# cserteGT3/RANSAC.jl

Measured on AMD Instinct MI355X. Metric: candidates_scored_per_sec, higher is better.
Workload: dtype f64; 1 GPU; cfg3: 10M-point 40-primitive cloud, 30% outliers, r=32 subsets, B=4096 candidates/GPU/step; points=10000000, subset_points=312500, score_mode=f64, parallelism=candidate-sharded x1, int32 sum all-reduce

## Files before the change

include/ransac_hip_diag.h:

```cpp
#ifndef RANSAC_HIP_DIAG_H
#define RANSAC_HIP_DIAG_H

#include "ransac_hip.h"

#ifdef __cplusplus
extern "C" {
#endif

int rh_dbg_cls_audit(rh_cloud *c, const rh_shape *shapes, int32_t b, const rh_params *p, double *out );
int rh_dbg_cls_soundness(rh_cloud *c, const rh_shape *shapes, int32_t b, const rh_params *p, uint64_t *out );
int rh_dbg_cls_soundness_tiles(rh_cloud *c, const rh_shape *shapes, int32_t b, const rh_params *p, uint64_t *out );
int rh_dbg_cls_soundness_nsig(rh_cloud *c, const rh_shape *shapes, int32_t b, const rh_params *p, uint64_t *out );
int rh_dbg_nsig(const rh_shape *shape, const rh_params *p, double M, double Nm, double Ln, int f32, uint32_t *mask_out ,
                const double *dirs, int64_t ndirs, int32_t *cells_out);
int rh_dbg_group_boxes(rh_cloud *c, double *out, int64_t cap, int64_t *ngroups_out);
int rh_dbg_cylbox(const rh_shape *shape, const rh_params *p, double M, double Nm, int f32, const double *boxes, int64_t n,
                  uint8_t *skip_out, uint8_t *ball_out, float *fields_out );
int rh_dbg_cls_round(const rh_shape *shape, const rh_params *p, double M, double Nm, int f32, int64_t n, const double *xyz,
                     const double *nrm, float *ua_out, float *ub_out, float *rec_out , double *dbg4_out );
int rh_dbg_conebox(const rh_shape *shape, const rh_params *p, double M, double Nm, int f32, const double *boxes, int64_t n,
                   uint8_t *skip_out, float *fields_out );
int rh_dbg_cls_cone(const rh_shape *shape, const rh_params *p, double M, double Nm, int f32, int64_t n, const double *xyz,
                    const double *nrm, int device, float *ua_out, float *ub_out, uint8_t *near_out, float *rec_out ,
                    double *dbg4_out );
int rh_dbg_oct_search_selftest(int64_t n, uint64_t seed, int64_t queries, int64_t *mismatches);

int rh_dbg_enabled_events(const uint8_t *events, int64_t nseq, int32_t len, uint16_t *answers);

int rh_dbg_s4_stats(rh_cloud *c, int mode, uint64_t *out );

typedef struct { int64_t slot; int32_t level; int32_t pad; rh_shape shape; } rh_dbg_cand;
int rh_dbg_sample_fit(rh_cloud *c, const rh_params *p, uint64_t seed, int64_t k0, int32_t n_iters, const double *P_or_null,
                      int32_t rank, int32_t world, rh_dbg_cand *out, int32_t cap, int32_t *n_out, uint64_t *draws_out,
                      int32_t *gave_up_out, int32_t *info_out );

int rh_dbg_wave_keys(const uint32_t *keys, const uint8_t *act, const int32_t *slot, int32_t n, int32_t nslots, int u32, int device,
                     int32_t *sum_out , int32_t *minlead_out , int32_t *scal_out );

#ifdef __cplusplus
}
#endif
#endif
```

ransac.jl_amd/_lib.py:

```python
import ctypes as C
import os

_HERE = os.path.dirname(os.path.abspath(__file__))
SO_PATH = os.path.join(_HERE, "libransac_hip.so")
SO_PATH_DIAG = os.path.join(_HERE, "libransac_hip_diag.so")
OPTION_UNSET = -(1 << 63)
SCORE_PATH = {"auto": 0, "brute": 1, "groups": 2}
REFIT_PATH = {"auto": 0, "scan": 1, "culled": 2}

PLANE, SPHERE, CYLINDER, CONE = 0, 1, 2, 3
KIND_NAMES = {PLANE: "plane", SPHERE: "sphere", CYLINDER: "cylinder", CONE: "cone"}
SCORE_INT64_WRAP, SCORE_F64 = 0, 1
S_LENGTHC, S_ALLCAND, S_NOFMINSET = 1, 2, 3
RH_OK, RH_E_INVALID, RH_E_NODEVICE, RH_E_NOMEM, RH_E_CAPACITY, RH_E_INTERNAL = 0, -1, -2, -3, -4, -5


class Shape(C.Structure):
    _fields_ = [("kind", C.c_int32), ("outwards", C.c_int32), ("v", C.c_double * 10)]


class Params(C.Structure):
    _fields_ = [
        ("eps", C.c_double * 4), ("alpha", C.c_double * 4), ("cos_alpha", C.c_double * 4),
        ("collin_threshold", C.c_double), ("parallelthrdeg", C.c_double), ("cos_parallelthr", C.c_double),
# ... 165 lines not shown
    "rh_mp_allgather": (C.c_int, [_vp, _vp, C.c_int64, _vp]),
    "rh_ransac_mp": (C.c_int, [_vp, C.POINTER(C.c_double), C.POINTER(C.c_double), C.POINTER(Params), C.POINTER(Rng), _vp, C.POINTER(Result)]),
    "rh_dev_free": (C.c_int, [_vp, _vp]),
    "rh_dev_upload": (C.c_int, [_vp, _vp, _vp, C.c_int64]),
    "rh_dev_download": (C.c_int, [_vp, _vp, _vp, C.c_int64]),
    "rh_octree_build": (C.c_int, [_dp, C.c_int64, C.POINTER(C.c_void_p)]),
    "rh_octree_build_f32": (C.c_int, [C.POINTER(C.c_float), C.c_int64, C.POINTER(C.c_void_p)]),
    "rh_octree_destroy": (C.c_int, [_vp]),
    "rh_octree_info": (C.c_int, [_vp, _i32p, _i32p, _i32p]),
    "rh_octree_findleaf": (C.c_int, [_vp, _dp, _i32p]),
    "rh_octree_getnthcell": (C.c_int, [_vp, C.c_int32, C.c_int32, _i32p]),
    "rh_octree_node_info": (C.c_int, [_vp, C.c_int32, _dp, _dp, _i32p, _i32p, _i32p, C.POINTER(C.c_int64)]),
    "rh_octree_node_points": (C.c_int, [_vp, C.c_int32, C.POINTER(C.c_int64), C.c_int64]),
    "rh_octree_cell_enabled": (C.c_int, [_vp, _vp, C.c_int32, C.POINTER(C.c_int64), C.c_int64, C.POINTER(C.c_int64)]),
    "rh_set_option": (C.c_int, [_vp, C.c_char_p, C.c_int64]),
    "rh_get_option": (C.c_int, [_vp, C.c_char_p, _i64p, _i32p]),
    "rh_score_launch_info": (C.c_int, [_vp, C.POINTER(C.c_int32)]),
    "rh_last_list_launch_ms": (C.c_int, [_vp, C.POINTER(C.c_float)]),
    "rh_build_variant": (C.c_int, []),
    "rh_cloud_create_ms": (C.c_int, [_vp, _dp]),
    "rh_comm_unique_id": (C.c_int, [_vp]),
    "rh_comm_create": (C.c_int, [_vp, C.c_int32, C.c_int32, _vp, C.POINTER(_vp)]),
    "rh_comm_destroy": (C.c_int, [_vp]),
    "rh_score_batch_allreduce_dev": (C.c_int, [_vp, _vp, _vp, C.c_int32, C.c_int32, C.c_int32, _pp, _vp]),
    "rh_comm_fence": (C.c_int, [_vp, _vp]),
    "rh_comm_sync": (C.c_int, [_vp]),
    "rh_shape_extents": (C.c_int, [_vp, _sp, C.c_int32, _i64p, _i64p, C.POINTER(Extent)]),
    "rh_shape_extents_dev": (C.c_int, [_vp, _vp, C.c_int32, _vp, _vp, C.c_int64, _vp]),
    "rh_result_extents": (C.c_int, [_vp, C.POINTER(Result), C.POINTER(Extent)]),
    "rh_assign_points": (C.c_int, [_dp, _dp, C.c_int64, _sp, C.c_int32, _pp, C.c_int32, C.c_int, _i32p, _dp, _i64p, _i64p, _i64p]),
    "rh_assign_points_f32": (C.c_int, [C.POINTER(C.c_float), C.POINTER(C.c_float), C.c_int64, _sp, C.c_int32, _pp, C.c_int32, C.c_int,
                                       _i32p, _dp, _i64p, _i64p, _i64p]),
    "rh_cloud_assign": (C.c_int, [_vp, _sp, C.c_int32, _pp, C.c_int32, _i32p, _dp, _i64p, _i64p, _i64p]),
    "rh_cloud_assign_dev": (C.c_int, [_vp, _vp, C.c_int32, _pp, C.c_int32, _vp, _vp, _vp, _vp, _vp]),
    "rh_estimate_normals": (C.c_int, [_dp, C.c_int64, C.POINTER(NormalsParams), _dp, C.c_int, _dp, _dp, _i32p]),
    "rh_estimate_normals_f32": (C.c_int, [C.POINTER(C.c_float), C.c_int64, C.POINTER(NormalsParams), C.POINTER(C.c_float),
                                          C.c_int, C.POINTER(C.c_float), C.POINTER(C.c_float), _i32p]),
    "rh_cluster": (C.c_int, [_dp, C.c_int64, C.POINTER(ClusterParams), C.c_int, _i32p, _u8p, C.c_int64, _i64p, _i64p, _i64p, _i64p,
                             C.POINTER(ClusterStats)]),
    "rh_cluster_f32": (C.c_int, [C.POINTER(C.c_float), C.c_int64, C.POINTER(ClusterParams), C.c_int, _i32p, _u8p, C.c_int64, _i64p,
                                 _i64p, _i64p, _i64p, C.POINTER(ClusterStats)]),
    "rh_orient_normals": (C.c_int, [_dp, _dp, C.c_int64, C.POINTER(OrientParams), C.c_int, _dp, _i32p, _i32p, C.POINTER(OrientStats)]),
    "rh_orient_normals_f32": (C.c_int, [C.POINTER(C.c_float), C.POINTER(C.c_float), C.c_int64, C.POINTER(OrientParams), C.c_int,
                                        C.POINTER(C.c_float), _i32p, _i32p, C.POINTER(OrientStats)]),
    "rh_voxel_downsample": (C.c_int, [_dp, _dp, C.c_int64, C.POINTER(VoxelParams), C.c_int, _dp, _dp, _i64p, _i32p, C.c_int64,
                                      _i32p, _i64p, _i64p]),
    "rh_voxel_downsample_f32": (C.c_int, [C.POINTER(C.c_float), C.POINTER(C.c_float), C.c_int64, C.POINTER(VoxelParams), C.c_int,
                                          C.POINTER(C.c_float), C.POINTER(C.c_float), _i64p, _i32p, C.c_int64, _i32p, _i64p, _i64p]),
    "rh_knn": (C.c_int, [_dp, C.c_int64, C.c_int32, C.c_double, C.c_int, _i32p, _dp, _i32p]),
    "rh_knn_f32": (C.c_int, [C.POINTER(C.c_float), C.c_int64, C.c_int32, C.c_double, C.c_int, _i32p, _dp, _i32p]),
    "rh_knn_query": (C.c_int, [_dp, C.c_int64, _dp, C.c_int64, C.c_int32, C.c_double, C.c_int, _i32p, _dp, _i32p]),
    "rh_knn_query_f32": (C.c_int, [C.POINTER(C.c_float), C.c_int64, C.POINTER(C.c_float), C.c_int64, C.c_int32, C.c_double, C.c_int,
                                   _i32p, _dp, _i32p]),
    "rh_cloud_distance": (C.c_int, [_dp, _dp, C.c_int64, _dp, C.c_int64, C.POINTER(DistanceParams), C.c_int, _dp, _i32p,
                                    C.POINTER(DistanceStats)]),
    "rh_cloud_distance_f32": (C.c_int, [C.POINTER(C.c_float), C.POINTER(C.c_float), C.c_int64, C.POINTER(C.c_float), C.c_int64,
                                        C.POINTER(DistanceParams), C.c_int, _dp, _i32p, C.POINTER(DistanceStats)]),
    "rh_register": (C.c_int, [_dp, _dp, C.c_int64, _dp, C.c_int64, C.POINTER(RegisterParams), _dp, C.c_int, _dp,
                              C.POINTER(RegisterResult), _i32p, _dp]),
    "rh_register_f32": (C.c_int, [C.POINTER(C.c_float), C.POINTER(C.c_float), C.c_int64, C.POINTER(C.c_float), C.c_int64,
                                  C.POINTER(RegisterParams), _dp, C.c_int, _dp, C.POINTER(RegisterResult), _i32p, _dp]),
    "rh_remove_outliers": (C.c_int, [_dp, C.c_int64, C.POINTER(OutlierParams), C.c_int, _u8p, _i32p, C.c_int64, _i64p, _dp,
                                     C.POINTER(OutlierStats)]),
    "rh_remove_outliers_f32": (C.c_int, [C.POINTER(C.c_float), C.c_int64, C.POINTER(OutlierParams), C.c_int, _u8p, _i32p,
                                         C.c_int64, _i64p, _dp, C.POINTER(OutlierStats)]),
}

class DbgCand(C.Structure):
    _fields_ = [("slot", C.c_int64), ("level", C.c_int32), ("pad", C.c_int32), ("shape", Shape)]


DIAG_SIGNATURES = {
    "rh_dbg_sample_fit": (C.c_int, [_vp, _pp, C.c_uint64, C.c_int64, C.c_int32, _dp, C.c_int32, C.c_int32, C.POINTER(DbgCand),
                                    C.c_int32, _i32p, _u64p, _i32p, _i32p]),
    "rh_dbg_cls_audit": (C.c_int, [_vp, _sp, C.c_int32, _pp, _dp]),
    "rh_dbg_cls_soundness": (C.c_int, [_vp, _sp, C.c_int32, _pp, C.POINTER(C.c_uint64)]),
    "rh_dbg_cls_soundness_tiles": (C.c_int, [_vp, _sp, C.c_int32, _pp, C.POINTER(C.c_uint64)]),
    "rh_dbg_cls_soundness_nsig": (C.c_int, [_vp, _sp, C.c_int32, _pp, C.POINTER(C.c_uint64)]),
    "rh_dbg_nsig": (C.c_int, [_sp, _pp, C.c_double, C.c_double, C.c_double, C.c_int, C.POINTER(C.c_uint32), _dp, C.c_int64, _i32p]),
    "rh_dbg_group_boxes": (C.c_int, [_vp, _dp, C.c_int64, C.POINTER(C.c_int64)]),
    "rh_dbg_cylbox": (C.c_int, [_sp, _pp, C.c_double, C.c_double, C.c_int, _dp, C.c_int64, C.POINTER(C.c_uint8), C.POINTER(C.c_uint8), C.POINTER(C.c_float)]),
    "rh_dbg_cls_round": (C.c_int, [_sp, _pp, C.c_double, C.c_double, C.c_int, C.c_int64, _dp, _dp, C.POINTER(C.c_float), C.POINTER(C.c_float),
                                   C.POINTER(C.c_float), _dp]),
    "rh_dbg_conebox": (C.c_int, [_sp, _pp, C.c_double, C.c_double, C.c_int, _dp, C.c_int64, C.POINTER(C.c_uint8), C.POINTER(C.c_float)]),
    "rh_dbg_cls_cone": (C.c_int, [_sp, _pp, C.c_double, C.c_double, C.c_int, C.c_int64, _dp, _dp, C.c_int, C.POINTER(C.c_float),
                                  C.POINTER(C.c_float), C.POINTER(C.c_uint8), C.POINTER(C.c_float), _dp]),
    "rh_dbg_oct_search_selftest": (C.c_int, [C.c_int64, C.c_uint64, C.c_int64, C.POINTER(C.c_int64)]),
    "rh_dbg_enabled_events": (C.c_int, [_u8p, C.c_int64, C.c_int32, C.POINTER(C.c_uint16)]),
    "rh_dbg_s4_stats": (C.c_int, [_vp, C.c_int, C.POINTER(C.c_uint64)]),
    "rh_dbg_wave_keys": (C.c_int, [C.POINTER(C.c_uint32), _u8p, _i32p, C.c_int32, C.c_int32, C.c_int, C.c_int, _i32p, _i32p, _i32p]),
}

_libs = {}


def variant():
    v = os.environ.get("RH_LIB_VARIANT", "product")
    if v not in ("product", "diag"):
        raise RuntimeError("RH_LIB_VARIANT=%r: expected 'product' or 'diag'" % v)
    return v


def _share_torch_hip_runtime():
    import sys
    if "torch" in sys.modules or os.environ.get("RH_SYSTEM_HIP"):
        return
    try:
        import importlib.util
        spec = importlib.util.find_spec("torch")
        if spec is None or not spec.submodule_search_locations:
            return
        path = os.path.join(list(spec.submodule_search_locations)[0], "lib", "libamdhip64.so")
        if os.path.exists(path):
            C.CDLL(path, mode=C.RTLD_GLOBAL)
    except (ImportError, OSError, ValueError):
        pass


def lib(which=None):
    which = which or variant()
    L = _libs.get(which)
    if L is None:
        path = SO_PATH if which == "product" else SO_PATH_DIAG
        if os.environ.get("RH_LIB_PATH"):
            path = os.environ["RH_LIB_PATH"]
        if not os.path.exists(path):
            raise RuntimeError(
                "%s is missing: the HIP extension has not been built and this package has no CPU "
                "fallback (build it with ransac.jl_amd/build.py)" % path)
        _share_torch_hip_runtime()
        L = C.CDLL(path)
        sigs = dict(SIGNATURES)
        if which == "diag":
            sigs.update(DIAG_SIGNATURES)
        for name, (res, args) in sigs.items():
            f = getattr(L, name)
            f.restype = res
            f.argtypes = args
        if L.rh_build_variant() != (1 if which == "diag" else 0):
            raise RuntimeError("%s is not the %s build" % (path, which))
        _libs[which] = L
    return L


def check(rc):
    if rc != RH_OK:
        raise RansacHipError(rc, lib().rh_last_error().decode("utf-8", "replace"))
    return rc
```

ransac.jl_amd/csrc/score4.hip:

```cpp
#include <stdio.h>
#include <stdlib.h>

#include <vector>

#include "rh_internal.h"
#ifdef RH_DIAG
#include "ransac_hip_diag.h"
#endif
#include "score_device.h"
#include "score4_device.h"
#include "wave_keys.h"

namespace {

using namespace rhdev;
using namespace rh4;

typedef float rh_f32x4 __attribute__((ext_vector_type(4)));
typedef float rh_f32x2 __attribute__((ext_vector_type(2)));
typedef unsigned long long rh_u64x2 __attribute__((ext_vector_type(2)));
typedef uint32_t rh_u32x4 __attribute__((ext_vector_type(4)));

constexpr int S4_TG = 4;
constexpr int S4_GB = 2;
// ... 48 lines not shown
    int64_t stcap;
};

#ifdef RH_DIAG
#define S4_STAT(stats, idx, val) do { const unsigned long long v_ = (unsigned long long)(val); if ((stats) != nullptr && (threadIdx.x & 63) == 0) atomicAdd((stats) + (idx), v_); } while (0)
#else
#define S4_STAT(stats, idx, val) do { } while (0)
#endif

template <int KIND> struct S4Fields { static constexpr int NBOX = KIND == RH_PLANE ? 8 : (KIND == RH_SPHERE ? 5 : (KIND == RH_CYLINDER ? 10 : 11)); };

static __device__ __forceinline__ bool nsig_meet(const float (&B)[RH_BOX_FIELDS], const rh_u32x4 gm)
{
    return (((__builtin_bit_cast(uint32_t, B[5]) & gm.x) | (__builtin_bit_cast(uint32_t, B[6]) & gm.y)) | (__builtin_bit_cast(uint32_t, B[7]) & gm.z)) != 0u;
}

#define RH4_CONST_AS __attribute__((address_space(4)))

static __device__ __forceinline__ int wave_shr1(int v) { return __builtin_amdgcn_update_dpp(0, v, 0x138, 0xf, 0xf, false); }
static __device__ __forceinline__ int wave_shl1(int v) { return __builtin_amdgcn_update_dpp(0, v, 0x130, 0xf, 0xf, false); }

static __device__ __forceinline__ int run_total(int v, int key, int lane)
{
    static_assert(S4_TG <= 4, "two steps cover runs of four");
    const int k1 = wave_shr1(key), u1 = wave_shr1(v);
    v += (lane >= 1 && k1 == key) ? u1 : 0;
    const int k2 = wave_shr1(k1), u2 = wave_shr1(wave_shr1(v));
    v += (lane >= 2 && k2 == key) ? u2 : 0;
    const int kn = wave_shl1(key);
    return (lane == 63 || kn != key) ? v : 0;
}

template <int KIND, int R, bool MASK, bool F32, bool LIST>
static __device__ __forceinline__ void
score4_batch(S4Shared<R, MASK, LIST> &sh, const int wv, const int lane, const int head, const int n, const int cbase, const double *__restrict__ pts,
             int64_t stride, const int64_t p0, const rh_prep *__restrict__ prep, const rh_cls *__restrict__ cls,
             const int32_t *__restrict__ orig, double eps, double cosa, int32_t *__restrict__ counts, const bool weird,
             uint64_t *__restrict__ masks, uint8_t *__restrict__ occ, const int64_t mstride, const int64_t g0, unsigned long long *__restrict__ stats)
{
    (void)stats;
    S4_STAT(stats, 24 * KIND + 8, 1);
    const bool act = lane < n;
    const uint32_t e = sh.plist[head + (act ? lane : 0)];
    const int g = (int)(e & S4_GM), ci = LIST ? (int)sh.ctab[e >> S4_GB] : cbase + (int)(e >> S4_GB);
    const rh_f32x4 *__restrict__ rowa = &sh.pa[g][0];
    const rh_f32x2 *__restrict__ rowb = &sh.pb[g][0];
    const rh_cls *__restrict__ rec = &cls[ci];
    int total = 0;
    uint64_t word = 0;
    int qbh = 0, qbn = 0;
    auto drain_b = [&](int k) {
        wave_lds_sync();
        const bool on = lane < k;
        const unsigned e2 = on ? sh.qb[wv][(qbh + lane) & 127] : 0u;
        const int slot = (int)(e2 >> 6);
        const uint32_t pe = sh.plist[head + slot];
        const int64_t gi = p0 + (int)(pe & S4_GM) * 64 + (int)(e2 & 63u);
        uint64_t r;
        if (F32) {
            const rh_prepf Pv = prepf_of<KIND>(prep[LIST ? (int)sh.ctab[pe >> S4_GB] : cbase + (int)(pe >> S4_GB)]);
            const rh_f32x4 a = sh.pa[pe & S4_GM][e2 & 63u];
            const rh_f32x2 b = sh.pb[pe & S4_GM][e2 & 63u];
            r = test_point<KIND>(Pv, a.x, a.y, a.z, a.w, b.x, b.y, eps, cosa);
        } else {
            const rh_prep Pv = prep[LIST ? (int)sh.ctab[pe >> S4_GB] : cbase + (int)(pe >> S4_GB)];
            r = test_point<KIND>(Pv, pts[gi], pts[stride + gi], pts[2 * stride + gi], pts[3 * stride + gi], pts[4 * stride + gi],
                                 pts[5 * stride + gi], eps, cosa);
        }
        S4_STAT(stats, 24 * KIND + (k == 64 ? 11 : 12), 1);
        S4_STAT(stats, 24 * KIND + 13, __popcll(r & (k >= 64 ? ~0ULL : ((1ULL << k) - 1ULL))));
        if (on && ((r >> lane) & 1ULL)) {
            atomicAdd(&sh.cntb[wv][slot], 1);
            if (MASK) atomicOr(&sh.maskb[wv][slot], 1ULL << (e2 & 63u));
        }
        qbh = (qbh + k) & 127;
        qbn -= k;
    };
    if (KIND != RH_CONE) {
        constexpr int NF = KIND == RH_PLANE ? 9 : (KIND == RH_SPHERE ? 8 : 11);
        rh_cls C;
#pragma unroll
        for (int f = 0; f < NF; f++) C.f[f] = rec->f[f];
        const bool exact_only = weird || is_nan_bits(rec->f[RH_CLS_FLAG]);
        uint32_t wlo = 0, whi = 0, umin = 0xffffffffu;
        auto point_u = [&](int j) {
            const rh_f32x4 a = rowa[j];
            const rh_f32x2 b = rowb[j];
            const float u = KIND == RH_PLANE ? cls_plane_u(C, a.x, a.y, a.z, a.w, b.x, b.y)
                                             : cls_round_u<KIND == RH_PLANE ? RH_SPHERE : KIND>(C, a.x, a.y, a.z, a.w, b.x, b.y);
            const uint32_t ub = __builtin_bit_cast(uint32_t, u);
            umin = umin < ub ? umin : ub;
            return ub;
        };
#pragma unroll 8
        for (int j = 0; j < 32; j++) wlo = __builtin_amdgcn_alignbit(wlo, point_u(j), 31);
#pragma unroll 8
        for (int j = 32; j < 64; j++) whi = __builtin_amdgcn_alignbit(whi, point_u(j), 31);
        if (MASK) { wlo = __brev(wlo); whi = __brev(whi); }
        const int cs = __popc(wlo) + __popc(whi);
        const bool amb = act && (umin <= 0x3f800000u || exact_only);
        total = (act && !amb) ? cs : 0;
        word = (act && !amb) ? (((uint64_t)whi << 32) | wlo) : 0ULL;
        uint64_t redo = WB(amb);
        S4_STAT(stats, 24 * KIND + 9, __popcll(redo));
        if (redo != 0) {
            sh.cntb[wv][lane] = 0;
            if (MASK) sh.maskb[wv][lane] = 0ULL;
            while (redo != 0) {
                const int k = __builtin_ctzll(redo);
                redo &= redo - 1;
                const uint32_t ek = __builtin_amdgcn_readlane(e, k);
                const int g2 = (int)(ek & S4_GM);
                const int ci2 = LIST ? __builtin_amdgcn_readfirstlane((int)sh.ctab[ek >> S4_GB]) : cbase + (int)(ek >> S4_GB);
                const RH4_CONST_AS rh_cls *rk = (const RH4_CONST_AS rh_cls *)(uintptr_t)&cls[ci2];
                rh_cls Ck;
#pragma unroll
                for (int f = 0; f < NF; f++) Ck.f[f] = rk->f[f];
                const bool xo = weird || is_nan_bits(rk->f[RH_CLS_FLAG]);
                const rh_f32x4 a = sh.pa[g2][lane];
                const rh_f32x2 b = sh.pb[g2][lane];
                const float u = KIND == RH_PLANE ? cls_plane_u(Ck, a.x, a.y, a.z, a.w, b.x, b.y)
                                                 : cls_round_u<KIND == RH_PLANE ? RH_SPHERE : KIND>(Ck, a.x, a.y, a.z, a.w, b.x, b.y);
                const uint64_t lg = sh.len[g2];
                const uint64_t sure = xo ? 0ULL : (WB(cls_sure(u)) & lg);
                const uint64_t und = xo ? lg : (WB(cls_undecided(u)) & lg);
                if (lane == k) { total = __popcll(sure); word = sure; }
                const bool has = (und >> lane) & 1ULL;
                const int rank = __builtin_amdgcn_mbcnt_hi((uint32_t)(und >> 32), __builtin_amdgcn_mbcnt_lo((uint32_t)und, 0));
                if (has) sh.qb[wv][(qbh + qbn + rank) & 127] = (uint16_t)((k << 6) | lane);
                qbn += __popcll(und);
                S4_STAT(stats, 24 * KIND + 10, __popcll(und));
                if (qbn >= 64) drain_b(64);
            }
            if (qbn > 0) drain_b(qbn);
            wave_lds_sync();
            total += sh.cntb[wv][lane];
            if (MASK) word |= sh.maskb[wv][lane];
        }
    } else {
        rh_cls C;
#pragma unroll
        for (int f = 0; f < 13; f++) C.f[f] = rec->f[f];
        const bool exact_only = weird || is_nan_bits(rec->f[RH_CLS_FLAG]);
        uint32_t slo = 0, shi = 0, mlo = 0, mhi = 0;
#pragma unroll 4
        for (int j = 0; j < 32; j++) {
            const rh_f32x4 a = rowa[j];
            const rh_f32x2 b = rowb[j];
            const float u = cls_cone_u(C, a.x, a.y, a.z, a.w, b.x, b.y);
            slo = __builtin_amdgcn_alignbit(slo, __builtin_bit_cast(uint32_t, u), 31);
            mlo = __builtin_amdgcn_alignbit(mlo, __builtin_bit_cast(uint32_t, u - 1.0f), 31);
        }
#pragma unroll 4
        for (int j = 0; j < 32; j++) {
            const rh_f32x4 a = rowa[32 + j];
            const rh_f32x2 b = rowb[32 + j];
            const float u = cls_cone_u(C, a.x, a.y, a.z, a.w, b.x, b.y);
            shi = __builtin_amdgcn_alignbit(shi, __builtin_bit_cast(uint32_t, u), 31);
            mhi = __builtin_amdgcn_alignbit(mhi, __builtin_bit_cast(uint32_t, u - 1.0f), 31);
        }
        mlo &= ~slo; mhi &= ~shi;
        slo = __brev(slo); shi = __brev(shi); mlo = __brev(mlo); mhi = __brev(mhi);
        const uint64_t lg = sh.len[g];
        uint64_t sure = exact_only ? 0ULL : ((((uint64_t)shi << 32) | slo) & lg);
        uint64_t mask = exact_only ? lg : ((((uint64_t)mhi << 32) | mlo) & lg);
        if (!act) { mask = 0; sure = 0; }
        sh.cntb[wv][lane] = 0;
        if (MASK) sh.maskb[wv][lane] = 0ULL;
        while (WB(mask != 0) != 0) {
            const bool has = mask != 0;
            const int j = has ? __builtin_ctzll(mask) : 0;
            mask &= mask - 1;
            const uint64_t mm = WB(has);
            const int rank = __builtin_amdgcn_mbcnt_hi((uint32_t)(mm >> 32), __builtin_amdgcn_mbcnt_lo((uint32_t)mm, 0));
            if (has) sh.qb[wv][(qbh + qbn + rank) & 127] = (uint16_t)((lane << 6) | j);
            qbn += __popcll(mm);
            S4_STAT(stats, 24 * KIND + 15, 1);
            S4_STAT(stats, 24 * KIND + 10, __popcll(mm));
            if (qbn >= 64) drain_b(64);
        }
        if (qbn > 0) drain_b(qbn);
        wave_lds_sync();
        total = sh.cntb[wv][lane] + __popcll(sure);
        if (MASK) word = sh.maskb[wv][lane] | sure;
    }
    if (MASK) {
        const bool nz = act && word != 0;
        const uint64_t nzm = WB(nz);
        if (nzm != 0) {
            const int keyp = wave_shr1(act ? ci : -1 - lane);
            const uint64_t starts = WB(lane == 0 || keyp != (act ? ci : -1 - lane));
            const uint64_t below = lane == 63 ? ~0ULL : ((2ULL << lane) - 1ULL);
            const int rs = 63 - __builtin_clzll(starts & below);
            const uint64_t after = lane == 63 ? 0ULL : (starts >> (lane + 1));
            const int re = after != 0 ? lane + __builtin_ctzll(after) : 63;
            const uint64_t runm = (re == 63 ? ~0ULL : ((2ULL << re) - 1ULL)) & ~((1ULL << rs) - 1ULL);
            const int tot = __popcll(nzm & runm);
            int base = 0;
            int64_t mrow = 0;
            if (nz || (lane == rs && tot > 0)) mrow = orig[ci];
            if (lane == rs && tot > 0) base = atomicAdd((int32_t *)occ + mrow, tot);
            base = __shfl(base, rs);
            if (nz) {
                const int rank = __popcll(nzm & runm & ((1ULL << lane) - 1ULL));
                rh_u64x2 ent;
                ent.x = (uint64_t)(g0 + g);
                ent.y = word;
                ((rh_u64x2 *)masks)[mrow * mstride + base + rank] = ent;
            }
        }
    }
    S4_STAT(stats, 24 * KIND + 14, __popcll(WB(act && total > 0)));
    const int v = run_total(act ? total : 0, act ? ci : -1 - lane, lane);
    if (v != 0) atomicAdd(&counts[orig[ci]], v);
// ... 991 lines not shown
        rh_cls C;
        float box[RH_BOX_FIELDS];
        cls_make(P, RH_PLANE, p->eps[RH_PLANE], p->cos_alpha[RH_PLANE], M, Nm, C, box, 1, nullptr, f32 != 0, Ln);
        for (int k = 0; k < 3; k++) mask_out[k] = __builtin_bit_cast(uint32_t, box[5 + k]);
    }
    for (int64_t i = 0; i < ndirs; i++) {
        uint32_t w[3];
        nsig_point_bits(dirs[3 * i], dirs[3 * i + 1], dirs[3 * i + 2], w);
        if ((w[0] & w[1] & w[2]) == 0xffffffffu) cells_out[i] = -2;
        else if ((w[0] | w[1] | w[2]) == 0u) cells_out[i] = -1;
        else cells_out[i] = nsig_cell(dirs[3 * i], dirs[3 * i + 1], dirs[3 * i + 2]);
    }
    return RH_OK;
}

extern "C" int rh_dbg_group_boxes(rh_cloud *c, double *out, int64_t cap, int64_t *ngroups_out)
{
    if (c == nullptr || ngroups_out == nullptr || cap < 0) { rh_set_error("rh_dbg_group_boxes: bad arguments"); return RH_E_INVALID; }
    *ngroups_out = c->gb == nullptr ? 0 : c->ngroups;
    if (out == nullptr || cap < *ngroups_out || *ngroups_out == 0) return RH_OK;
    RH_HIP(hipSetDevice(c->device));
    std::vector<double> h((size_t)c->ngroups * 6);
    const double *gb = c->gb;
    for (int k = 0; k < 6; k++)
        RH_HIP(hipMemcpyAsync(h.data() + (size_t)k * c->ngroups, gb + (int64_t)k * c->ng_pad, sizeof(double) * (size_t)c->ngroups, hipMemcpyDeviceToHost, c->stream));
    RH_HIP(hipStreamSynchronize(c->stream));
    for (int64_t g = 0; g < c->ngroups; g++)
        for (int k = 0; k < 6; k++) out[6 * g + k] = h[(size_t)k * c->ngroups + g];
    return RH_OK;
}

extern "C" int rh_dbg_cylbox(const rh_shape *shape, const rh_params *p, double M, double Nm, int f32, const double *boxes, int64_t n,
                             uint8_t *skip_out, uint8_t *ball_out, float *fields_out)
{
    if (shape == nullptr || p == nullptr || n < 0 || (n > 0 && (boxes == nullptr || skip_out == nullptr || ball_out == nullptr))) {
        rh_set_error("rh_dbg_cylbox: bad arguments");
        return RH_E_INVALID;
    }
    if (shape->kind != RH_CYLINDER) { rh_set_error("rh_dbg_cylbox: cylinders only"); return RH_E_INVALID; }
    rh_prep P;
    rh_prep_host(*shape, &P);
    rh_cls C;
    float box[RH_BOX_FIELDS];
    cls_make(P, RH_CYLINDER, p->eps[RH_CYLINDER], p->cos_alpha[RH_CYLINDER], M, Nm, C, box, 1, nullptr, f32 != 0);
    if (fields_out != nullptr)
        for (int k = 0; k < RH_BOX_FIELDS; k++) fields_out[k] = box[k];
    for (int64_t i = 0; i < n; i++) {
        float o[8];
        box_to_f32(boxes + 6 * i, boxes + 6 * i + 3, o);
        rh_box32 G;
        G.cx = o[0]; G.cy = o[1]; G.cz = o[2]; G.hx = o[3]; G.hy = o[4]; G.hz = o[5]; G.hr = o[6];
        skip_out[i] = cyl_box_skip32<true>(box, G) ? 1 : 0;
        ball_out[i] = cyl_box_skip32<false>(box, G) ? 1 : 0;
    }
    return RH_OK;
}

extern "C" int rh_dbg_cls_round(const rh_shape *shape, const rh_params *p, double M, double Nm, int f32, int64_t n, const double *xyz,
                                const double *nrm, float *ua_out, float *ub_out, float *rec_out, double *dbg4_out)
{
    if (shape == nullptr || p == nullptr || n < 0 || (n > 0 && (xyz == nullptr || nrm == nullptr || ua_out == nullptr || ub_out == nullptr))) {
        rh_set_error("rh_dbg_cls_round: bad arguments");
        return RH_E_INVALID;
    }
    if (shape->kind != RH_SPHERE && shape->kind != RH_CYLINDER) { rh_set_error("rh_dbg_cls_round: spheres and cylinders only"); return RH_E_INVALID; }
    rh_prep P;
    rh_prep_host(*shape, &P);
    rh_cls C;
    double d4[4] = { 0, 0, 0, 0 };
    cls_make(P, shape->kind, p->eps[shape->kind], p->cos_alpha[shape->kind], M, Nm, C, nullptr, 0, d4, f32 != 0);
    if (rec_out != nullptr)
        for (int k = 0; k < 16; k++) rec_out[k] = C.f[k];
    if (dbg4_out != nullptr)
        for (int k = 0; k < 4; k++) dbg4_out[k] = d4[k];
    for (int64_t i = 0; i < n; i++) {
        const float x = (float)xyz[3 * i], y = (float)xyz[3 * i + 1], z = (float)xyz[3 * i + 2];
        const float nx = (float)nrm[3 * i], ny = (float)nrm[3 * i + 1], nz = (float)nrm[3 * i + 2];
        if (shape->kind == RH_SPHERE) cls_round_ab<RH_SPHERE>(C, x, y, z, nx, ny, nz, ua_out[i], ub_out[i]);
        else cls_round_ab<RH_CYLINDER>(C, x, y, z, nx, ny, nz, ua_out[i], ub_out[i]);
    }
    return RH_OK;
}

extern "C" int rh_dbg_conebox(const rh_shape *shape, const rh_params *p, double M, double Nm, int f32, const double *boxes, int64_t n,
                              uint8_t *skip_out, float *fields_out)
{
    if (shape == nullptr || p == nullptr || n < 0 || (n > 0 && (boxes == nullptr || skip_out == nullptr))) {
        rh_set_error("rh_dbg_conebox: bad arguments");
        return RH_E_INVALID;
    }
    if (shape->kind != RH_CONE) { rh_set_error("rh_dbg_conebox: cones only"); return RH_E_INVALID; }
    rh_prep P;
    rh_prep_host(*shape, &P);
    rh_cls C;
    float box[RH_BOX_FIELDS];
    cls_make(P, RH_CONE, p->eps[RH_CONE], p->cos_alpha[RH_CONE], M, Nm, C, box, 1, nullptr, f32 != 0);
    if (fields_out != nullptr)
        for (int k = 0; k < RH_BOX_FIELDS; k++) fields_out[k] = box[k];
    for (int64_t i = 0; i < n; i++) {
        float o[8];
        box_to_f32(boxes + 6 * i, boxes + 6 * i + 3, o);
        rh_box32 G;
        G.cx = o[0]; G.cy = o[1]; G.cz = o[2]; G.hx = o[3]; G.hy = o[4]; G.hz = o[5]; G.hr = o[6];
        skip_out[i] = cone_box_skip32(box, G) ? 1 : 0;
    }
    return RH_OK;
}

extern "C" int rh_dbg_cls_cone(const rh_shape *shape, const rh_params *p, double M, double Nm, int f32, int64_t n, const double *xyz,
                               const double *nrm, int device, float *ua_out, float *ub_out, uint8_t *near_out, float *rec_out, double *dbg4_out)
{
    if (shape == nullptr || p == nullptr || n < 0 || n > (int64_t)1 << 24 ||
        (n > 0 && (xyz == nullptr || nrm == nullptr || ua_out == nullptr || ub_out == nullptr || near_out == nullptr))) {
        rh_set_error("rh_dbg_cls_cone: bad arguments");
        return RH_E_INVALID;
    }
    if (shape->kind != RH_CONE) { rh_set_error("rh_dbg_cls_cone: cones only"); return RH_E_INVALID; }
    rh_prep P;
    rh_prep_host(*shape, &P);
    rh_cls C;
    double d4[4] = { 0, 0, 0, 0 };
    cls_make(P, RH_CONE, p->eps[RH_CONE], p->cos_alpha[RH_CONE], M, Nm, C, nullptr, 0, d4, f32 != 0);
    if (rec_out != nullptr)
        for (int k = 0; k < 16; k++) rec_out[k] = C.f[k];
    if (dbg4_out != nullptr)
        for (int k = 0; k < 4; k++) dbg4_out[k] = d4[k];
    if (n == 0) return RH_OK;
    std::vector<float> h((size_t)n * 6);
    for (int64_t i = 0; i < n; i++)
        for (int k = 0; k < 3; k++) {
            h[(size_t)(k * n + i)] = (float)xyz[3 * i + k];
            h[(size_t)((3 + k) * n + i)] = (float)nrm[3 * i + k];
        }
    RH_HIP(hipSetDevice(device));
    rh_dev<float> d_p, d_a, d_b;
    rh_dev<uint8_t> d_n;
    RH_TRY(d_p.alloc(n * 6));
    RH_TRY(d_a.alloc(n));
    RH_TRY(d_b.alloc(n));
    RH_TRY(d_n.alloc(n));
    RH_HIP(hipMemcpy(d_p, h.data(), sizeof(float) * (size_t)n * 6, hipMemcpyHostToDevice));
    hipLaunchKernelGGL(cls_cone_dbg_kernel, dim3((unsigned)cdiv4(n, 256)), dim3(256), 0, 0, C, (const float *)d_p, n, (float *)d_a, (float *)d_b, (uint8_t *)d_n);
    RH_HIP(hipGetLastError());
    RH_HIP(hipMemcpy(ua_out, d_a, sizeof(float) * (size_t)n, hipMemcpyDeviceToHost));
    RH_HIP(hipMemcpy(ub_out, d_b, sizeof(float) * (size_t)n, hipMemcpyDeviceToHost));
    RH_HIP(hipMemcpy(near_out, d_n, (size_t)n, hipMemcpyDeviceToHost));
    return RH_OK;
}

#endif

#ifdef RH_DIAG
extern "C" int rh_dbg_s4_stats(rh_cloud *c, int mode, uint64_t *out)
{
    if (c == nullptr || mode < 0 || mode > 2) { rh_set_error("rh_dbg_s4_stats: bad arguments"); return RH_E_INVALID; }
    RH_HIP(hipSetDevice(c->device));
    RH_HIP(hipStreamSynchronize(c->stream));
    if (mode == 1) {
        if (c->s4_stats == nullptr) RH_TRY(c->s4_stats.alloc(128));
        RH_HIP(hipMemset(c->s4_stats, 0, sizeof(unsigned long long) * 128));
    } else if (mode == 2) {
        c->s4_stats.reset();
    } else if (out != nullptr) {
        for (int i = 0; i < 128; i++) out[i] = 0;
        if (c->s4_stats != nullptr) RH_HIP(hipMemcpy(out, c->s4_stats, sizeof(unsigned long long) * 128, hipMemcpyDeviceToHost));
    }
// ... 43 lines not shown
```

ransac.jl_amd/csrc/score4_device.h:

```cpp
#pragma once

#include "rh_internal.h"

namespace rh4 {

constexpr double RH_CLS_U = 5.9604644775390625e-08;
constexpr double RH_CLS_SAFETY = 2.0;
constexpr double RH_CLS_BIG = 1048576.0;

struct rh_cls {
    float f[16];
};
constexpr int RH_CLS_FLAG = 15;

constexpr int RH_BOX_FIELDS = 11;
constexpr float RH_CONE_ALPHA = (float)((RH_CLS_SAFETY * 49.0 + 64.0) * RH_CLS_U);

__host__ __device__ inline bool cls_fin(double v) { return v - v == 0.0; }

__host__ __device__ inline float cls_dn(double v) { return (float)(v - fabs(v) * (2.0 * RH_CLS_U) - 1e-37); }
__host__ __device__ inline float cls_up(double v) { return (float)(v + fabs(v) * (2.0 * RH_CLS_U) + 1e-37); }

__host__ __device__ inline double cls_slack64(const rh_prep &P, double M) { return 1e-9 * ((1.0 + M) + P.f[11]); }

// ... 241 lines not shown
            bx[10] = f32cloud ? 1e-3f : RH_CONE_ALPHA;
        }
    }
    if (!ok) o.f[RH_CLS_FLAG] = fnan;
    if (box != nullptr)
        for (int i = 0; i < RH_BOX_FIELDS; i++) box[(int64_t)i * bstride] = bx[i];
}

__host__ __device__ inline void box_to_f32(const double c[3], const double h[3], float o[8])
{
    double h2 = 0;
    for (int k = 0; k < 3; k++) {
        const float cf = (float)c[k];
        const double hh = (h[k] + fabs(c[k] - (double)cf)) * (1.0 + 4.0 * RH_CLS_U) + 1e-37;
        const float hf = cls_up(hh);
        o[k] = cf;
        o[3 + k] = hf;
        h2 += (double)hf * (double)hf;
    }
    o[6] = cls_up(sqrt(h2));
    o[7] = 0.0f;
}

#ifdef __HIPCC__
#define WB4(cond) __builtin_amdgcn_ballot_w64(cond)

struct rh_box32 { float cx, cy, cz, hx, hy, hz, hr; };

template <bool SUPPORT>
static __host__ __device__ __forceinline__ bool cyl_box_skip32(const float (&B)[RH_BOX_FIELDS], const rh_box32 &G)
{
    const float tx = G.cx - B[3], ty = G.cy - B[4], tz = G.cz - B[5];
    const float sd = __builtin_fmaf(B[2], tz, __builtin_fmaf(B[1], ty, B[0] * tx));
    const float qx = __builtin_fmaf(-B[0], sd, tx), qy = __builtin_fmaf(-B[1], sd, ty), qz = __builtin_fmaf(-B[2], sd, tz);
    const float rho2 = __builtin_fmaf(qz, qz, __builtin_fmaf(qy, qy, qx * qx));
    const float lip = B[8] * G.hr * 1.000001f;
    const float X = B[6] + lip, Y = B[7] - lip;
    const float X2 = X > 0.0f ? X * X * 1.000001f : (X <= 0.0f ? 0.0f : X);
    bool skip = (rho2 * 0.999999f > X2) | ((Y > 0.0f) & (rho2 * 1.000001f < Y * Y));
    if (SUPPORT) {
        const float aq = __builtin_fmaf(B[2], qz, __builtin_fmaf(B[1], qy, B[0] * qx));
        const float gx = __builtin_fmaf(-B[0], aq, qx), gy = __builtin_fmaf(-B[1], aq, qy), gz = __builtin_fmaf(-B[2], aq, qz);
        const float s = __builtin_fmaf(__builtin_fabsf(gz), G.hz, __builtin_fmaf(__builtin_fabsf(gy), G.hy, __builtin_fabsf(gx) * G.hx));
        const float w = __builtin_fmaf(rho2, 0.999999f, -s);
        skip |= (w > 0.0f) & (w * w > B[9] * rho2);
    }
    return skip;
}

static __host__ __device__ __forceinline__ bool cone_box_skip32(const float (&B)[RH_BOX_FIELDS], const rh_box32 &G)
{
    const float tx = G.cx - B[0], ty = G.cy - B[1], tz = G.cz - B[2];
    const float tt = __builtin_fmaf(tz, tz, __builtin_fmaf(ty, ty, tx * tx));
    const float h = __builtin_fmaf(tz, B[5], __builtin_fmaf(ty, B[4], tx * B[3]));
    const float rho2 = __builtin_fmaf(-h, h, tt);
    const float s2 = __builtin_fmaf(B[10], tt, B[9]);
    const float e = __builtin_fmaf(G.hr, B[7], B[8]) * 1.000001f;
    const float uu = B[6] * h;
    const float lo = uu - e, hi = uu + e;
    const float hi2 = __builtin_fmaf(hi, hi, s2), lo2 = __builtin_fmaf(lo, lo, -s2);
    return (rho2 > s2) & ((hi <= 0.0f) | (rho2 > hi2) | ((lo > 0.0f) & (rho2 < lo2)));
}

template <int KIND>
static __device__ __forceinline__ bool box_skip32(const float (&B)[RH_BOX_FIELDS], const rh_box32 &G)
{
    if (KIND == RH_PLANE) {
        const float d = __builtin_fmaf(B[2], G.cz, __builtin_fmaf(B[1], G.cy, __builtin_fmaf(B[0], G.cx, B[3])));
        const float ext = __builtin_fmaf(__builtin_fabsf(B[2]), G.hz, __builtin_fmaf(__builtin_fabsf(B[1]), G.hy, __builtin_fmaf(__builtin_fabsf(B[0]), G.hx, B[4])));
        return __builtin_fabsf(d) > ext;
    }
    if (KIND == RH_SPHERE) {
        const float ax = __builtin_fabsf(G.cx - B[0]), ay = __builtin_fabsf(G.cy - B[1]), az = __builtin_fabsf(G.cz - B[2]);
        const float nx = fmaxf(ax - G.hx, 0.0f), ny = fmaxf(ay - G.hy, 0.0f), nz = fmaxf(az - G.hz, 0.0f);
        const float fx = ax + G.hx, fy = ay + G.hy, fz = az + G.hz;
        const float dmin2 = __builtin_fmaf(nz, nz, __builtin_fmaf(ny, ny, nx * nx));
        const float dmax2 = __builtin_fmaf(fz, fz, __builtin_fmaf(fy, fy, fx * fx)) * 1.000001f;
        return (dmin2 * 0.999999f > B[3]) | (dmax2 < B[4]);
    }
    if (KIND == RH_CYLINDER) return cyl_box_skip32<true>(B, G);
    return cone_box_skip32(B, G);
}

static __device__ __forceinline__ void cls_plane_ab(const rh_cls &C, float x, float y, float z, float nx, float ny, float nz, float &ua, float &ub)
{
    ua = __builtin_fmaf(C.f[2], nz, __builtin_fmaf(C.f[1], ny, __builtin_fmaf(C.f[0], nx, C.f[3])));
    const float d = __builtin_fmaf(C.f[6], z, __builtin_fmaf(C.f[5], y, __builtin_fmaf(C.f[4], x, C.f[7])));
    ub = __builtin_fabsf(d) - C.f[8];
}
static __device__ __forceinline__ float cls_plane_u(const rh_cls &C, float x, float y, float z, float nx, float ny, float nz)
{
    float a, b;
    cls_plane_ab(C, x, y, z, nx, ny, nz, a, b);
    return fmaxf(a, b);
}

template <int KIND>
static __host__ __device__ __forceinline__ void cls_round_ab(const rh_cls &C, float x, float y, float z, float nx, float ny, float nz, float &ua, float &ub)
{
    float qx, qy, qz;
    constexpr int b = KIND == RH_SPHERE ? 3 : 6;
    if (KIND == RH_SPHERE) {
        qx = x - C.f[0]; qy = y - C.f[1]; qz = z - C.f[2];
    } else {
        const float tx = x - C.f[3], ty = y - C.f[4], tz = z - C.f[5];
        const float sd = __builtin_fmaf(C.f[2], tz, __builtin_fmaf(C.f[1], ty, C.f[0] * tx));
        qx = __builtin_fmaf(-C.f[0], sd, tx); qy = __builtin_fmaf(-C.f[1], sd, ty); qz = __builtin_fmaf(-C.f[2], sd, tz);
    }
    const float n2 = __builtin_fmaf(qz, qz, __builtin_fmaf(qy, qy, qx * qx));
    const float qn = __builtin_fmaf(qz, nz, __builtin_fmaf(qy, ny, qx * nx));
    ua = __builtin_fmaf(__builtin_fabsf(n2 - C.f[b]), C.f[b + 1], C.f[b + 2]);
    ub = __builtin_fmaf(qn * __builtin_fabsf(qn), C.f[b + 3], __builtin_fmaf(n2, C.f[b + 4], 0.5f));
}
template <int KIND>
static __device__ __forceinline__ float cls_round_u(const rh_cls &C, float x, float y, float z, float nx, float ny, float nz)
{
    float a, b;
    cls_round_ab<KIND>(C, x, y, z, nx, ny, nz, a, b);
    return fmaxf(a, b);
}

static __device__ __forceinline__ void cls_cone_ab(const rh_cls &C, float x, float y, float z, float nx, float ny, float nz, float &ua, float &ub,
                                                   bool &near_axis)
{
    const float wx = x - C.f[0], wy = y - C.f[1], wz = z - C.f[2];
    const float h = __builtin_fmaf(wz, C.f[5], __builtin_fmaf(wy, C.f[4], wx * C.f[3]));
    const float qx = __builtin_fmaf(-C.f[3], h, wx), qy = __builtin_fmaf(-C.f[4], h, wy), qz = __builtin_fmaf(-C.f[5], h, wz);
    const float n2 = __builtin_fmaf(qz, qz, __builtin_fmaf(qy, qy, qx * qx));
    const float rho = n2 * __builtin_amdgcn_rsqf(n2);
    const float D = __builtin_fmaf(C.f[6], rho, C.f[7] * h);
    ua = __builtin_fabsf(D) - C.f[8];
    const float qn = __builtin_fmaf(qz, nz, __builtin_fmaf(qy, ny, qx * nx));
    const float an = __builtin_fmaf(C.f[5], nz, __builtin_fmaf(C.f[4], ny, C.f[3] * nx));
    ub = __builtin_fmaf(qn, C.f[9], __builtin_fmaf(rho, __builtin_fmaf(an, C.f[10], C.f[11]), 0.5f));
    const float tt = __builtin_fmaf(h, h, n2);
    near_axis = !(n2 > __builtin_fmaf(RH_CONE_ALPHA, tt, C.f[12]));
}
static __device__ __forceinline__ float cls_cone_u(const rh_cls &C, float x, float y, float z, float nx, float ny, float nz)
{
    float a, b;
    bool near_axis;
    cls_cone_ab(C, x, y, z, nx, ny, nz, a, b, near_axis);
    return near_axis ? 0.5f : fmaxf(a, b);
}
static __device__ __forceinline__ bool cls_sure(float u) { return (__builtin_bit_cast(uint32_t, u) >> 31) != 0; }
static __device__ __forceinline__ bool cls_undecided(float u) { return __builtin_bit_cast(uint32_t, u) <= 0x3f800000u; }
#endif

}
```

Before: 77.64 million candidates/s.

## Pack two-bit classifier state per point to skip recomputation in ambiguous redo loop

Classifier coefficients are doubled so each point's u2 value carries both the sure and undecided decisions in its top two bits. These bits are packed into four 32-bit words per lane. The redo path for ambiguous lanes now reads the precomputed undecided mask via readlane instead of reloading coefficients and re-evaluating the classifier for every ambiguous candidate. The cost is extra bit-compression work on every lane and a changed numeric threshold scheme whose soundness depends on the doubling being exact. Host debug hooks are added to check the new encoding.

```diff
diff --git a/include/ransac_hip_diag.h b/include/ransac_hip_diag.h
--- a/include/ransac_hip_diag.h
+++ b/include/ransac_hip_diag.h
@@ -18,6 +18,10 @@
                   uint8_t *skip_out, uint8_t *ball_out, float *fields_out );
 int rh_dbg_cls_round(const rh_shape *shape, const rh_params *p, double M, double Nm, int f32, int64_t n, const double *xyz,
                      const double *nrm, float *ua_out, float *ub_out, float *rec_out , double *dbg4_out );
+int rh_dbg_books2(const float *u2, int64_t nseq, int32_t *sure_count_out, uint64_t *sure_word_out, uint64_t *und_word_out,
+                  uint8_t *any_und_out);
+int rh_dbg_cls_u2(const rh_shape *shape, const rh_params *p, double M, double Nm, int f32, int64_t n, const double *xyz,
+                  const double *nrm, float *u_out, float *u2_out, float *rec_out );
 int rh_dbg_conebox(const rh_shape *shape, const rh_params *p, double M, double Nm, int f32, const double *boxes, int64_t n,
                    uint8_t *skip_out, float *fields_out );
 int rh_dbg_cls_cone(const rh_shape *shape, const rh_params *p, double M, double Nm, int f32, int64_t n, const double *xyz,
diff --git a/ransac.jl_amd/_lib.py b/ransac.jl_amd/_lib.py
--- a/ransac.jl_amd/_lib.py
+++ b/ransac.jl_amd/_lib.py
@@ -271,6 +271,9 @@
     "rh_dbg_cylbox": (C.c_int, [_sp, _pp, C.c_double, C.c_double, C.c_int, _dp, C.c_int64, C.POINTER(C.c_uint8), C.POINTER(C.c_uint8), C.POINTER(C.c_float)]),
     "rh_dbg_cls_round": (C.c_int, [_sp, _pp, C.c_double, C.c_double, C.c_int, C.c_int64, _dp, _dp, C.POINTER(C.c_float), C.POINTER(C.c_float),
                                    C.POINTER(C.c_float), _dp]),
+    "rh_dbg_books2": (C.c_int, [C.POINTER(C.c_float), C.c_int64, _i32p, _u64p, _u64p, _u8p]),
+    "rh_dbg_cls_u2": (C.c_int, [_sp, _pp, C.c_double, C.c_double, C.c_int, C.c_int64, _dp, _dp, C.POINTER(C.c_float), C.POINTER(C.c_float),
+                                C.POINTER(C.c_float)]),
     "rh_dbg_conebox": (C.c_int, [_sp, _pp, C.c_double, C.c_double, C.c_int, _dp, C.c_int64, C.POINTER(C.c_uint8), C.POINTER(C.c_float)]),
     "rh_dbg_cls_cone": (C.c_int, [_sp, _pp, C.c_double, C.c_double, C.c_int, C.c_int64, _dp, _dp, C.c_int, C.POINTER(C.c_float),
                                   C.POINTER(C.c_float), C.POINTER(C.c_uint8), C.POINTER(C.c_float), _dp]),
diff --git a/ransac.jl_amd/csrc/score4.hip b/ransac.jl_amd/csrc/score4.hip
--- a/ransac.jl_amd/csrc/score4.hip
+++ b/ransac.jl_amd/csrc/score4.hip
@@ -154,54 +154,38 @@
 #pragma unroll
         for (int f = 0; f < NF; f++) C.f[f] = rec->f[f];
         const bool exact_only = weird || is_nan_bits(rec->f[RH_CLS_FLAG]);
-        uint32_t wlo = 0, whi = 0, umin = 0xffffffffu;
-        auto point_u = [&](int j) {
-            const rh_f32x4 a = rowa[j];
-            const rh_f32x2 b = rowb[j];
-            const float u = KIND == RH_PLANE ? cls_plane_u(C, a.x, a.y, a.z, a.w, b.x, b.y)
-                                             : cls_round_u<KIND == RH_PLANE ? RH_SPHERE : KIND>(C, a.x, a.y, a.z, a.w, b.x, b.y);
-            const uint32_t ub = __builtin_bit_cast(uint32_t, u);
-            umin = umin < ub ? umin : ub;
-            return ub;
-        };
+        cls_double<KIND>(C);
+        uint32_t w[4] = { 0u, 0u, 0u, 0u };
+#pragma unroll
+        for (int q = 0; q < 4; q++) {
 #pragma unroll 8
-        for (int j = 0; j < 32; j++) wlo = __builtin_amdgcn_alignbit(wlo, point_u(j), 31);
-#pragma unroll 8
-        for (int j = 32; j < 64; j++) whi = __builtin_amdgcn_alignbit(whi, point_u(j), 31);
-        if (MASK) { wlo = __brev(wlo); whi = __brev(whi); }
-        const int cs = __popc(wlo) + __popc(whi);
-        const bool amb = act && (umin <= 0x3f800000u || exact_only);
-        total = (act && !amb) ? cs : 0;
-        word = (act && !amb) ? (((uint64_t)whi << 32) | wlo) : 0ULL;
+            for (int j = 0; j < 16; j++) {
+                const rh_f32x4 a = rowa[16 * q + j];
+                const rh_f32x2 b = rowb[16 * q + j];
+                w[q] = books2_push(w[q], cls_u2<KIND>(C, a.x, a.y, a.z, a.w, b.x, b.y));
+            }
+        }
+        const bool amb = act && (exact_only || books2_any_undecided(w));
+        total = (act && !exact_only) ? books2_sure_count(w) : 0;
+        if (MASK) word = (act && !exact_only) ? books2_sure64(w) : 0ULL;
         uint64_t redo = WB(amb);
         S4_STAT(stats, 24 * KIND + 9, __popcll(redo));
         if (redo != 0) {
+            const uint64_t lg = sh.len[g];
+            const uint64_t und = exact_only ? lg : (books2_und64(w) & lg);
+            const uint32_t undlo = (uint32_t)und, undhi = (uint32_t)(und >> 32);
             sh.cntb[wv][lane] = 0;
             if (MASK) sh.maskb[wv][lane] = 0ULL;
             while (redo != 0) {
                 const int k = __builtin_ctzll(redo);
                 redo &= redo - 1;
-                const uint32_t ek = __builtin_amdgcn_readlane(e, k);
-                const int g2 = (int)(ek & S4_GM);
-                const int ci2 = LIST ? __builtin_amdgcn_readfirstlane((int)sh.ctab[ek >> S4_GB]) : cbase + (int)(ek >> S4_GB);
-                const RH4_CONST_AS rh_cls *rk = (const RH4_CONST_AS rh_cls *)(uintptr_t)&cls[ci2];
-                rh_cls Ck;
-#pragma unroll
-                for (int f = 0; f < NF; f++) Ck.f[f] = rk->f[f];
-                const bool xo = weird || is_nan_bits(rk->f[RH_CLS_FLAG]);
-                const rh_f32x4 a = sh.pa[g2][lane];
-                const rh_f32x2 b = sh.pb[g2][lane];
-                const float u = KIND == RH_PLANE ? cls_plane_u(Ck, a.x, a.y, a.z, a.w, b.x, b.y)
-                                                 : cls_round_u<KIND == RH_PLANE ? RH_SPHERE : KIND>(Ck, a.x, a.y, a.z, a.w, b.x, b.y);
-                const uint64_t lg = sh.len[g2];
-                const uint64_t sure = xo ? 0ULL : (WB(cls_sure(u)) & lg);
-                const uint64_t und = xo ? lg : (WB(cls_undecided(u)) & lg);
-                if (lane == k) { total = __popcll(sure); word = sure; }
-                const bool has = (und >> lane) & 1ULL;
-                const int rank = __builtin_amdgcn_mbcnt_hi((uint32_t)(und >> 32), __builtin_amdgcn_mbcnt_lo((uint32_t)und, 0));
+                const uint32_t ulo = __builtin_amdgcn_readlane(undlo, k), uhi = __builtin_amdgcn_readlane(undhi, k);
+                const uint64_t uk = ((uint64_t)uhi << 32) | ulo;
+                const bool has = (uk >> lane) & 1ULL;
+                const int rank = __builtin_amdgcn_mbcnt_hi(uhi, __builtin_amdgcn_mbcnt_lo(ulo, 0));
                 if (has) sh.qb[wv][(qbh + qbn + rank) & 127] = (uint16_t)((k << 6) | lane);
-                qbn += __popcll(und);
-                S4_STAT(stats, 24 * KIND + 10, __popcll(und));
+                qbn += __popcll(uk);
+                S4_STAT(stats, 24 * KIND + 10, __popcll(uk));
                 if (qbn >= 64) drain_b(64);
             }
             if (qbn > 0) drain_b(qbn);
@@ -1359,6 +1343,54 @@
     return RH_OK;
 }
 
+extern "C" int rh_dbg_books2(const float *u2, int64_t nseq, int32_t *sure_count_out, uint64_t *sure_word_out, uint64_t *und_word_out,
+                             uint8_t *any_und_out)
+{
+    if (nseq < 0 || (nseq > 0 && (u2 == nullptr || sure_count_out == nullptr || sure_word_out == nullptr || und_word_out == nullptr || any_und_out == nullptr))) {
+        rh_set_error("rh_dbg_books2: bad arguments");
+        return RH_E_INVALID;
+    }
+    for (int64_t s = 0; s < nseq; s++) {
+        uint32_t w[4] = { 0u, 0u, 0u, 0u };
+        for (int q = 0; q < 4; q++)
+            for (int j = 0; j < 16; j++) w[q] = books2_push(w[q], u2[64 * s + 16 * q + j]);
+        sure_count_out[s] = books2_sure_count(w);
+        sure_word_out[s] = books2_sure64(w);
+        und_word_out[s] = books2_und64(w);
+        any_und_out[s] = books2_any_undecided(w) ? 1 : 0;
+    }
+    return RH_OK;
+}
+
+extern "C" int rh_dbg_cls_u2(const rh_shape *shape, const rh_params *p, double M, double Nm, int f32, int64_t n, const double *xyz,
+                             const double *nrm, float *u_out, float *u2_out, float *rec_out)
+{
+    if (shape == nullptr || p == nullptr || n < 0 || (n > 0 && (xyz == nullptr || nrm == nullptr || u_out == nullptr || u2_out == nullptr))) {
+        rh_set_error("rh_dbg_cls_u2: bad arguments");
+        return RH_E_INVALID;
+    }
+    const int kind = shape->kind;
+    if (kind != RH_PLANE && kind != RH_SPHERE && kind != RH_CYLINDER) { rh_set_error("rh_dbg_cls_u2: planes, spheres and cylinders only"); return RH_E_INVALID; }
+    rh_prep P;
+    rh_prep_host(*shape, &P);
+    rh_cls C;
+    cls_make(P, kind, p->eps[kind], p->cos_alpha[kind], M, Nm, C, nullptr, 0, nullptr, f32 != 0);
+    if (rec_out != nullptr)
+        for (int k = 0; k < 16; k++) rec_out[k] = C.f[k];
+    rh_cls D = C;
+    if (kind == RH_PLANE) cls_double<RH_PLANE>(D);
+    else if (kind == RH_SPHERE) cls_double<RH_SPHERE>(D);
+    else cls_double<RH_CYLINDER>(D);
+    for (int64_t i = 0; i < n; i++) {
+        const float x = (float)xyz[3 * i], y = (float)xyz[3 * i + 1], z = (float)xyz[3 * i + 2];
+        const float nx = (float)nrm[3 * i], ny = (float)nrm[3 * i + 1], nz = (float)nrm[3 * i + 2];
+        if (kind == RH_PLANE) { u_out[i] = cls_plane_u(C, x, y, z, nx, ny, nz); u2_out[i] = cls_u2<RH_PLANE>(D, x, y, z, nx, ny, nz); }
+        else if (kind == RH_SPHERE) { u_out[i] = cls_round_u<RH_SPHERE>(C, x, y, z, nx, ny, nz); u2_out[i] = cls_u2<RH_SPHERE>(D, x, y, z, nx, ny, nz); }
+        else { u_out[i] = cls_round_u<RH_CYLINDER>(C, x, y, z, nx, ny, nz); u2_out[i] = cls_u2<RH_CYLINDER>(D, x, y, z, nx, ny, nz); }
+    }
+    return RH_OK;
+}
+
 extern "C" int rh_dbg_conebox(const rh_shape *shape, const rh_params *p, double M, double Nm, int f32, const double *boxes, int64_t n,
                               uint8_t *skip_out, float *fields_out)
 {
diff --git a/ransac.jl_amd/csrc/score4_device.h b/ransac.jl_amd/csrc/score4_device.h
--- a/ransac.jl_amd/csrc/score4_device.h
+++ b/ransac.jl_amd/csrc/score4_device.h
@@ -347,13 +347,13 @@
     return cone_box_skip32(B, G);
 }
 
-static __device__ __forceinline__ void cls_plane_ab(const rh_cls &C, float x, float y, float z, float nx, float ny, float nz, float &ua, float &ub)
+static __host__ __device__ __forceinline__ void cls_plane_ab(const rh_cls &C, float x, float y, float z, float nx, float ny, float nz, float &ua, float &ub)
 {
     ua = __builtin_fmaf(C.f[2], nz, __builtin_fmaf(C.f[1], ny, __builtin_fmaf(C.f[0], nx, C.f[3])));
     const float d = __builtin_fmaf(C.f[6], z, __builtin_fmaf(C.f[5], y, __builtin_fmaf(C.f[4], x, C.f[7])));
     ub = __builtin_fabsf(d) - C.f[8];
 }
-static __device__ __forceinline__ float cls_plane_u(const rh_cls &C, float x, float y, float z, float nx, float ny, float nz)
+static __host__ __device__ __forceinline__ float cls_plane_u(const rh_cls &C, float x, float y, float z, float nx, float ny, float nz)
 {
     float a, b;
     cls_plane_ab(C, x, y, z, nx, ny, nz, a, b);
@@ -361,7 +361,8 @@
 }
 
 template <int KIND>
-static __host__ __device__ __forceinline__ void cls_round_ab(const rh_cls &C, float x, float y, float z, float nx, float ny, float nz, float &ua, float &ub)
+static __host__ __device__ __forceinline__ void cls_round_ab(const rh_cls &C, float x, float y, float z, float nx, float ny, float nz, float &ua, float &ub,
+                                                            const float half = 0.5f)
 {
     float qx, qy, qz;
     constexpr int b = KIND == RH_SPHERE ? 3 : 6;
@@ -375,13 +376,13 @@
     const float n2 = __builtin_fmaf(qz, qz, __builtin_fmaf(qy, qy, qx * qx));
     const float qn = __builtin_fmaf(qz, nz, __builtin_fmaf(qy, ny, qx * nx));
     ua = __builtin_fmaf(__builtin_fabsf(n2 - C.f[b]), C.f[b + 1], C.f[b + 2]);
-    ub = __builtin_fmaf(qn * __builtin_fabsf(qn), C.f[b + 3], __builtin_fmaf(n2, C.f[b + 4], 0.5f));
+    ub = __builtin_fmaf(qn * __builtin_fabsf(qn), C.f[b + 3], __builtin_fmaf(n2, C.f[b + 4], half));
 }
 template <int KIND>
-static __device__ __forceinline__ float cls_round_u(const rh_cls &C, float x, float y, float z, float nx, float ny, float nz)
+static __host__ __device__ __forceinline__ float cls_round_u(const rh_cls &C, float x, float y, float z, float nx, float ny, float nz, const float half = 0.5f)
 {
     float a, b;
-    cls_round_ab<KIND>(C, x, y, z, nx, ny, nz, a, b);
+    cls_round_ab<KIND>(C, x, y, z, nx, ny, nz, a, b, half);
     return fmaxf(a, b);
 }
 
@@ -410,6 +411,60 @@
 }
 static __device__ __forceinline__ bool cls_sure(float u) { return (__builtin_bit_cast(uint32_t, u) >> 31) != 0; }
 static __device__ __forceinline__ bool cls_undecided(float u) { return __builtin_bit_cast(uint32_t, u) <= 0x3f800000u; }
+
+template <int KIND>
+static __host__ __device__ __forceinline__ void cls_double(rh_cls &C)
+{
+    constexpr int lo = KIND == RH_PLANE ? 0 : (KIND == RH_SPHERE ? 4 : 7), hi = KIND == RH_PLANE ? 9 : (KIND == RH_SPHERE ? 8 : 11);
+#pragma unroll
+    for (int f = lo; f < hi; f++) C.f[f] = C.f[f] + C.f[f];
+}
+template <int KIND>
+static __host__ __device__ __forceinline__ float cls_u2(const rh_cls &C, float x, float y, float z, float nx, float ny, float nz)
+{
+    if (KIND == RH_PLANE) return cls_plane_u(C, x, y, z, nx, ny, nz);
+    return cls_round_u<KIND == RH_PLANE ? RH_SPHERE : KIND>(C, x, y, z, nx, ny, nz, 1.0f);
+}
+static __host__ __device__ __forceinline__ uint32_t books2_push(uint32_t w, float u2)
+{
+    const uint32_t b = __builtin_bit_cast(uint32_t, u2);
+#ifdef __HIP_DEVICE_COMPILE__
+    return __builtin_amdgcn_alignbit(w, b, 30);
+#else
+    return (w << 2) | (b >> 30);
 #endif
-
-}
+}
+constexpr uint32_t RH_BOOKS2_SIGN = 0xAAAAAAAAu;
+static __host__ __device__ __forceinline__ int books2_sure_count(const uint32_t (&w)[4])
+{
+    return (__builtin_popcount(w[0] & RH_BOOKS2_SIGN) + __builtin_popcount(w[1] & RH_BOOKS2_SIGN)) +
+           (__builtin_popcount(w[2] & RH_BOOKS2_SIGN) + __builtin_popcount(w[3] & RH_BOOKS2_SIGN));
+}
+static __host__ __device__ __forceinline__ uint32_t books2_und_bits(uint32_t w) { return ~(w | (w << 1)) & RH_BOOKS2_SIGN; }
+static __host__ __device__ __forceinline__ bool books2_any_undecided(const uint32_t (&w)[4])
+{
+    return (((books2_und_bits(w[0]) | books2_und_bits(w[1])) | books2_und_bits(w[2])) | books2_und_bits(w[3])) != 0u;
+}
+static __host__ __device__ __forceinline__ uint32_t books2_compress(uint32_t x)
+{
+    x = __builtin_bitreverse32(x);
+    x = (x | (x >> 1)) & 0x33333333u;
+    x = (x | (x >> 2)) & 0x0f0f0f0fu;
+    x = (x | (x >> 4)) & 0x00ff00ffu;
+    return (x | (x >> 8)) & 0x0000ffffu;
+}
+static __host__ __device__ __forceinline__ uint64_t books2_und64(const uint32_t (&w)[4])
+{
+    const uint32_t lo = books2_compress(books2_und_bits(w[0])) | (books2_compress(books2_und_bits(w[1])) << 16);
+    const uint32_t hi = books2_compress(books2_und_bits(w[2])) | (books2_compress(books2_und_bits(w[3])) << 16);
+    return ((uint64_t)hi << 32) | lo;
+}
+static __host__ __device__ __forceinline__ uint64_t books2_sure64(const uint32_t (&w)[4])
+{
+    const uint32_t lo = books2_compress(w[0] & RH_BOOKS2_SIGN) | (books2_compress(w[1] & RH_BOOKS2_SIGN) << 16);
+    const uint32_t hi = books2_compress(w[2] & RH_BOOKS2_SIGN) | (books2_compress(w[3] & RH_BOOKS2_SIGN) << 16);
+    return ((uint64_t)hi << 32) | lo;
+}
+#endif
+
+}
```

New measurement: 81.70 million candidates/s, median of 6. 5.2% higher.
